# ugadiarov-la-phystech-edu/OCRL

Measured on AMD Instinct MI355X. Metric: images/sec (node) SLATE pretrain 128x128, 6 slots, 3 iters, higher is better.
Workload: dtype f32

## Files before the change

include/ocrl_hip.h:

```cpp
#ifndef OCRL_HIP_H
#define OCRL_HIP_H
#include <stddef.h>

#ifdef __cplusplus
extern "C" {
#endif

#define OCRL_ABI_VERSION 5

const char* ocrl_last_error(void);
int ocrl_abi_version(void);

typedef struct ocrl_slate ocrl_slate;
typedef struct ocrl_slate_config {
    int obs_size, obs_channels;
    int vocab_size, d_model;
    int cnn_hidden;
    int num_slots, num_iterations, slot_size, mlp_hidden;
    int num_dec_blocks, num_dec_heads;
    float dropout;
    int max_batch;
    int use_bcdec;
    int hard;
    int num_slot_heads;
// ... 77 lines not shown
    int accumulate;
} ocrl_conv_wgrad_desc;
size_t ocrl_conv_wgrad_desc_size(void);
int ocrl_conv2d_bwd_weight_ex(const ocrl_conv_wgrad_desc* d, float* ws, size_t ws_floats, void* stream);
int ocrl_layernorm_fwd(const float* x, const float* gamma, const float* beta, float* y, float* mean, float* rstd, long long R, int F, void* stream);
int ocrl_layernorm_bwd(const float* dy, const float* x, const float* mean, const float* rstd, const float* gamma, float* dx, float* dgb,
                       long long R, int F, float* ws, size_t ws_floats, void* stream);

int ocrl_sa_input_plan(long long R, int out[3]);
int ocrl_sa_input_fwd(const float* e4, const float* gamma, const float* beta, const float* W0, const float* b0, const float* W2, const float* b2,
                      float* mean, float* rstd, float* h1, float* x, long long R, int max_wgs, void* stream);
int ocrl_sa_input_bwd(const float* dx, const float* h1, const float* e4, const float* mean, const float* rstd, const float* gamma, const float* beta,
                      const float* W0, const float* W2, float* de4, float* dW0, float* db0, float* dW2, float* db2, float* dgamma, float* dbeta,
                      long long R, int max_wgs, float* ws, size_t ws_floats, void* stream);

int ocrl_attention_fwd(const float* q, const float* k, const float* v, float* o, float* lse, int B, int T, int d, int h, int ld,
                       float p, unsigned long long seed, unsigned site, void* stream);
int ocrl_attention_bwd(const float* q, const float* k, const float* v, const float* o, const float* lse, const float* dO,
                       float* dq, float* dk, float* dv, float* delta, int B, int T, int d, int h, int ld,
                       float p, unsigned long long seed, unsigned site, void* stream);

int ocrl_obs_u8_to_f32(const unsigned char* obs_hwc, float* obs_chw, int B, int H, int W, int C, void* stream);

int ocrl_prof_enable(unsigned tag_mask);
int ocrl_prof_collect(double* ms, long long* count, int ntags);

size_t ocrl_slot_attention_ws_floats(int B, int K, int D, int H, int I);
int ocrl_slot_attention_fwd(const float* x, const float* slots0, const float* const* w, float* slots, float* attn, int B, int N, int K, int D,
                            int H, int I, float* ws, size_t ws_floats, void* stream);
int ocrl_slot_attention_bwd(const float* x, const float* dslots, float* dx, float* dslots0, float* const* dw, int B, int N, int K, int D, int H,
// ... 179 lines not shown
```

ocrl_amd/_lib.py:

```python
import ctypes
import os
from ctypes import POINTER, c_char_p, c_float, c_int, c_longlong, c_size_t, c_uint, c_ulonglong, c_void_p

_HERE = os.path.dirname(os.path.abspath(__file__))
LIB_PATH = os.environ.get("OCRL_HIP_LIB") or os.path.join(_HERE, "libocrl_hip.so")
_lib = None


class SlateConfig(ctypes.Structure):
    _fields_ = [(n, c_int) for n in ("obs_size", "obs_channels", "vocab_size", "d_model", "cnn_hidden", "num_slots",
                                      "num_iterations", "slot_size", "mlp_hidden", "num_dec_blocks", "num_dec_heads")] + \
               [("dropout", c_float), ("max_batch", c_int), ("use_bcdec", c_int), ("hard", c_int), ("num_slot_heads", c_int)]


class IodineConfig(ctypes.Structure):
    _fields_ = [(n, c_int) for n in ("obs_size", "obs_channels", "slot_size", "num_iterations", "num_slots")] + \
               [("sigma", c_float), ("beta", c_float), ("layer_norm", c_int), ("ref_mlp_hidden", c_int), ("max_batch", c_int)]


class GemmDesc(ctypes.Structure):
    _fields_ = [("A", c_void_p), ("B", c_void_p), ("C", c_void_p)] + \
               [(n, c_int) for n in ("M", "N", "K", "lda", "ldb", "ldc", "akc", "bkc", "batch", "batch_inner")] + \
               [(n, c_longlong) for n in ("sA", "sB", "sC", "sAi", "sBi", "sCi")] + \
               [("splitk", c_int), ("alpha", c_float), ("bias", c_void_p), ("relu", c_int),
# ... 122 lines not shown
    L.ocrl_conv2d_wgrad_ws_floats.restype = c_size_t
    L.ocrl_conv2d_bwd_weight.argtypes = [p, p, p, p, c_int, c_int, c_int, c_int, c_int, c_int, p, c_size_t, p]
    L.ocrl_conv_desc_size.restype = c_size_t
    L.ocrl_conv_wgrad_desc_size.restype = c_size_t
    for name, cls in (("ocrl_conv_desc", ConvDesc), ("ocrl_conv_wgrad_desc", ConvWgradDesc)):
        n = getattr(L, name + "_size")()
        if n != ctypes.sizeof(cls):
            raise RuntimeError(f"libocrl_hip.so: {name} is {n} bytes, this binding's {cls.__name__} {ctypes.sizeof(cls)}")
    L.ocrl_conv2d_ex.argtypes = [POINTER(ConvDesc), p, c_size_t, p]
    L.ocrl_conv2d_bwd_weight_ex.argtypes = [POINTER(ConvWgradDesc), p, c_size_t, p]
    L.ocrl_layernorm_fwd.argtypes = [p, p, p, p, p, p, c_longlong, c_int, p]
    L.ocrl_layernorm_bwd.argtypes = [p, p, p, p, p, p, p, c_longlong, c_int, p, c_size_t, p]
    L.ocrl_sa_input_plan.argtypes = [c_longlong, POINTER(c_int * 3)]
    L.ocrl_sa_input_fwd.argtypes = [p] * 11 + [c_longlong, c_int, p]
    L.ocrl_sa_input_bwd.argtypes = [p] * 16 + [c_longlong, c_int, p, c_size_t, p]
    L.ocrl_attention_fwd.argtypes = [p, p, p, p, p, c_int, c_int, c_int, c_int, c_int, c_float, c_ulonglong, c_uint, p]
    L.ocrl_attention_bwd.argtypes = [p, p, p, p, p, p, p, p, p, p, c_int, c_int, c_int, c_int, c_int, c_float, c_ulonglong, c_uint, p]
    L.ocrl_obs_u8_to_f32.argtypes = [p, p, c_int, c_int, c_int, c_int, p]
    L.ocrl_prof_enable.argtypes = [c_uint]
    L.ocrl_prof_collect.argtypes = [POINTER(ctypes.c_double * 8), POINTER(c_longlong * 8), c_int]
    L.ocrl_iodine_create.argtypes = [POINTER(IodineConfig), POINTER(p)]
    L.ocrl_iodine_destroy.argtypes = [p]
    L.ocrl_iodine_destroy.restype = None
    L.ocrl_iodine_param_count.argtypes = [p]
    L.ocrl_iodine_param_info.argtypes = [p, c_int, c_char_p, c_int, POINTER(c_int * 4), POINTER(c_int), POINTER(c_longlong), POINTER(c_longlong)]
    L.ocrl_iodine_flat_size.argtypes = [p]
    L.ocrl_iodine_flat_size.restype = c_longlong
    L.ocrl_iodine_workspace_bytes.argtypes = [p]
    L.ocrl_iodine_workspace_bytes.restype = c_size_t
    L.ocrl_iodine_bind.argtypes = [p, p, p, p, p, p, c_size_t]
# ... 113 lines not shown
```

ocrl_amd/csrc/capi.cpp:

```cpp
#include <stdarg.h>
#include <stdint.h>
#include <string.h>

#include <new>

#include "../../include/ocrl_hip.h"
#include "iodine_model.h"
#include "slate_model.h"

static thread_local char g_err[512] = "";

void ocrl_set_error(const char* fmt, ...) {
    va_list ap;
    va_start(ap, fmt);
    vsnprintf(g_err, sizeof g_err, fmt, ap);
    va_end(ap);
}

template <class M>
struct Handle {
    using Model = M;
    M* m = nullptr;
};
struct ocrl_slate : Handle<SlateModel> {};
// ... 272 lines not shown
    if (!out || R <= 0) { ocrl_set_error("ocrl_sa_input_plan: needs R > 0 and an output array"); return 1; }
    sa_input_plan(R, 0, out);
    return 0;
}
int ocrl_sa_input_fwd(const float* e4, const float* gamma, const float* beta, const float* W0, const float* b0, const float* W2, const float* b2,
                      float* mean, float* rstd, float* h1, float* x, long long R, int max_wgs, void* stream) {
    return sa_input_fwd_launch(e4, gamma, beta, W0, b0, W2, b2, mean, rstd, nullptr, h1, x, R, max_wgs, ST(stream));
}
int ocrl_sa_input_bwd(const float* dx, const float* h1, const float* e4, const float* mean, const float* rstd, const float* gamma, const float* beta,
                      const float* W0, const float* W2, float* de4, float* dW0, float* db0, float* dW2, float* db2, float* dgamma, float* dbeta,
                      long long R, int max_wgs, float* ws, size_t ws_floats, void* stream) {
    return sa_input_bwd_launch(dx, h1, e4, mean, rstd, gamma, beta, W0, W2, de4, dW0, db0, dW2, db2, dgamma, dbeta, R, max_wgs, ws, ws_floats,
                               ST(stream));
}

int ocrl_attention_fwd(const float* q, const float* k, const float* v, float* o, float* lse, int B, int T, int d, int h, int ld, float p,
                       unsigned long long seed, unsigned site, void* stream) {
    AttnArgs a;
    a.q = q; a.k = k; a.v = v; a.o = o; a.lse = lse; a.B = B; a.T = T; a.d = d; a.h = h; a.ld = ld; a.p = p; a.seed = seed; a.site = site;
    return attn_launch(a, 0, ST(stream));
}
int ocrl_attention_bwd(const float* q, const float* k, const float* v, const float* o, const float* lse, const float* dO, float* dq,
                       float* dk, float* dv, float* delta, int B, int T, int d, int h, int ld, float p, unsigned long long seed,
                       unsigned site, void* stream) {
    AttnArgs a;
    a.q = q; a.k = k; a.v = v; a.o = const_cast<float*>(o); a.lse = const_cast<float*>(lse); a.B = B; a.T = T; a.d = d; a.h = h; a.ld = ld;
    a.p = p; a.seed = seed; a.site = site; a.dO = dO; a.dq = dq; a.dk = dk; a.dv = dv; a.delta = delta;
    return attn_launch(a, 1, ST(stream));
}

// ... 37 lines not shown
```

ocrl_amd/csrc/kernels.h:

```cpp
#pragma once
#include "common.h"
#include "../../include/ocrl_hip.h"

enum { PROF_CONV5 = 0, PROF_CONV_OTHER = 1, PROF_WGRAD = 2, PROF_GEMM = 3, PROF_SA_FWD = 4, PROF_SA_BWD = 5, PROF_ATTN_FWD = 6, PROF_ATTN_BWD = 7, PROF_NTAGS = 8 };
int prof_begin(int tag, hipStream_t st);
void prof_end(int idx, hipStream_t st);

struct GemmArgs {
    const float* A = nullptr;
    const float* B = nullptr;
    float* C = nullptr;
    int M = 0, N = 0, K = 0;
    int lda = 0, ldb = 0, ldc = 0;
    int akc = 1, bkc = 1;
    int batch = 1;
    int batch_inner = 1;
    long long sA = 0, sB = 0, sC = 0;
    long long sAi = 0, sBi = 0, sCi = 0;
    int splitk = 1;
    long long sCsplit = 0;
    float alpha = 1.f;
    const float* bias = nullptr;
    int relu = 0;
    float drop_p = 0.f;
// ... 198 lines not shown
int patchify4_launch(const float* in, float* out, int B, int C, int S, hipStream_t st);
int pixel_shuffle_launch(const float* in, float* out, int B, int h, int w, int Cout, int forward, const float* mask, hipStream_t st);
int layernorm_fwd_launch(const float* x, const float* g, const float* b, float* y, float* mean, float* rstd, long long R, int F, hipStream_t st);
int layernorm_bwd_launch(const float* dy, const float* x, const float* mean, const float* rstd, const float* g, float* dx,
                         float* dgb, long long R, int F, int accumulate_dx, int accumulate_dgb, float* ws, size_t ws_floats, hipStream_t st);
int colsum_launch(const float* X, long long ld, float* out, long long R, int F, int accumulate, float scale, float* ws, size_t ws_floats, hipStream_t st);

#define SA_INPUT_SLAB (2 * 4096 + 4 * 64)
void sa_input_plan(long long R, int max_wgs, int out[3]);
int sa_input_fwd_launch(const float* e4, const float* gamma, const float* beta, const float* W0, const float* b0, const float* W2, const float* b2,
                        float* mean, float* rstd, float* ln0, float* h1, float* x, long long R, int max_wgs, hipStream_t st);
int sa_input_bwd_launch(const float* dx, const float* h1, const float* e4, const float* mean, const float* rstd, const float* gamma, const float* beta,
                        const float* W0, const float* W2, float* de4, float* dW0, float* db0, float* dW2, float* db2, float* dgamma, float* dbeta,
                        long long R, int max_wgs, float* ws, size_t ws_floats, hipStream_t st);
int reduce_partials_launch(const float* part, int n, float* out, float scale, int accumulate, hipStream_t st);
int mse_launch(const float* obs, const float* recon, float* drecon, float* out, int B, int C, int H, int W, float* ws, size_t ws_floats, hipStream_t st);
int gumbel_softmax_launch(const float* raw, const float* e1, const float* e2, float* z, int* tokens, long long R, int V, float tau,
                          unsigned long long seed, hipStream_t st, float* zst = nullptr);
int softmax_bwd_rows_launch(const float* z, float* d, long long R, int V, float scale, hipStream_t st);
int softmax_stat_combine_launch(const float* stat, int nseg, long long R, float* lse, const float* hstat, const int* hidx, int* tokens,
                                const float* pred, int ldp, const int* tok, float* out, float scale, float* ws, size_t ws_floats, hipStream_t st,
                                const float* cdf_scores = nullptr, int cdf_V = 0, float cdf_tau = 1.f, unsigned long long cdf_seed = 0);
int exp_rows_launch(const float* y, const float* lse, float* z, long long R, int V, hipStream_t st);
int rowdot_bias64_launch(const float* g, const float* act, const float* bias, long long R, float* out, hipStream_t st);
int embed_fwd_launch(const int* tokens, const float* dict, const float* bos, const float* pe, float* out, int B, int T, int d, float p,
                     unsigned long long seed, hipStream_t st);
size_t embed_bwd_ws_floats(long long BT, int V, int d);
int embed_bwd_launch(float* g, const int* tokens, float* ddict, int B, int T, int V, int d, float p, unsigned long long seed, float* ws,
                     size_t ws_floats, hipStream_t st);
int dropout_apply_launch(const float* x, float* y, long long n, float p, unsigned long long seed, unsigned site, hipStream_t st);
// ... 177 lines not shown
```

ocrl_amd/csrc/slate_model.cpp:

```cpp
#include "slate_model.h"

#include <stdlib.h>
#include <functional>
#include <utility>

#include <math.h>
#include <stdarg.h>
#include <string.h>

static std::string fmt(const char* f, ...) {
    char buf[256];
    va_list ap;
    va_start(ap, f);
    vsnprintf(buf, sizeof buf, f, ap);
    va_end(ap);
    return buf;
}

SlateModel::SlateModel(const SlateConfig& c) : cfg(c) {
    S = c.obs_size; E = S / 4; T = E * E; N = S * S; V = c.vocab; d = c.d_model; C = c.cnn_hidden;
    K = c.num_slots; I = c.num_iters; D = c.slot_size; H = c.mlp_hidden; NB = c.num_blocks; NH = c.num_heads;
    DH = d / NH; Bmax = c.max_batch; SH = c.slot_heads > 0 ? c.slot_heads : 1;
    const int ch = c.obs_channels;
    add_param("_dvae._encoder.0.m.weight", {64, ch, 4, 4}, 0); add_param("_dvae._encoder.0.m.bias", {64}, 0);
// ... 229 lines not shown
            OCRL_HIP(hipEventCreateWithFlags(&ev_fork_, hipEventDisableTiming));
            OCRL_HIP(hipEventCreateWithFlags(&ev_join_, hipEventDisableTiming));
            OCRL_HIP(hipEventCreateWithFlags(&ev_tokens_, hipEventDisableTiming));
            const char* w = getenv("OCRL_DW_SIDE");
            dw_mode_ = (overlap_mode_ >= 3 && !cfg.use_bcdec) ? (w ? atoi(w) : 2) : 0;
            if (dw_mode_) {
                for (hipEvent_t& ev : ev_dw_) OCRL_HIP(hipEventCreateWithFlags(&ev, hipEventDisableTiming));
                OCRL_HIP(hipEventCreateWithFlags(&ev_join2_, hipEventDisableTiming));
                if (dw_mode_ == 2) OCRL_HIP(hipStreamCreateWithFlags(&side2_, hipStreamNonBlocking));
            }
        }
    }
    {
        const char* e = getenv("OCRL_SA_INPUT");
        sa_input_ = e ? atoi(e) : 1;
    }
    {
        const char* e = getenv("OCRL_XATTN");
        xattn_ = !cfg.use_bcdec && xattn_supported(K, d, NH) && (e ? atoi(e) != 0 : true);
        if (!cfg.use_bcdec && xa_zero_floats_) OCRL_HIP(hipMemset(xa_zero_base_, 0, xa_zero_floats_ * sizeof(float)));
    }
    RC(posgrid_launch(gridT_, S, 0));
    RC(fill_launch(recon_, (long long)Bmax * N * 4, 0.f, 0));
    const SaWts wo = sa_wts_layout(C, D, H);
    const std::string sa = "_slotattn.slot_attention.";
    std::vector<PackEntry> ent;
    auto e = [&](const std::string& name, int rows, int cols, int off, int tr) {
        PackEntry x; x.src = P(name); x.rows = rows; x.cols = cols; x.dst_off = off; x.transpose = tr;
        ent.push_back(x);
    };
// ... 151 lines not shown
        a.A = zraw_; a.B = P("_dvae._decoder.0.m.weight"); a.C = dd0_; a.M = (int)BT; a.N = 64; a.K = V; a.lda = V; a.ldb = V; a.ldc = 64;
        a.bias = P("_dvae._decoder.0.m.bias"); a.relu = 1; a.a_mode = 2; a.x_lse = zlse_;
        RC(gemm_launch(a, st));
    } else {
    if (!zin) zin = zdec_;
    RC(lin_fwd(zin, V, P("_dvae._decoder.0.m.weight"), P("_dvae._decoder.0.m.bias"), dd0_, 64, BT, 64, V, 1, nullptr, 0, 0.f, 0, st));
    }
    RC(conv_layer_fwd(dd0_, dw_fwd_[0], P("_dvae._decoder.1.m.bias"), dd1_, B, E, E, 3, 64, 1, nullptr, nullptr, st));
    RC(lin_fwd(dd1_, 64, P("_dvae._decoder.2.m.weight"), P("_dvae._decoder.2.m.bias"), dd2_, 64, BT, 64, 64, 1, nullptr, 0, 0.f, 0, st));
    RC(lin_fwd(dd2_, 64, P("_dvae._decoder.3.m.weight"), P("_dvae._decoder.3.m.bias"), dd3_, 64, BT, 64, 64, 1, nullptr, 0, 0.f, 0, st));
    RC(lin_fwd(dd3_, 64, P("_dvae._decoder.4.m.weight"), P("_dvae._decoder.4.m.bias"), dd4_, 256, BT, 256, 64, 1, nullptr, 0, 0.f, 0, st));
    RC(pixel_shuffle_launch(dd4_, ps1_, B, E, E, 64, 1, nullptr, st));
    RC(conv_layer_fwd(ps1_, dw_fwd_[1], P("_dvae._decoder.6.m.bias"), dd6_, B, 2 * E, 2 * E, 3, 64, 1, nullptr, nullptr, st));
    RC(lin_fwd(dd6_, 64, P("_dvae._decoder.7.m.weight"), P("_dvae._decoder.7.m.bias"), dd7_, 64, 4 * BT, 64, 64, 1, nullptr, 0, 0.f, 0, st));
    RC(lin_fwd(dd7_, 64, P("_dvae._decoder.8.m.weight"), P("_dvae._decoder.8.m.bias"), dd8_, 64, 4 * BT, 64, 64, 1, nullptr, 0, 0.f, 0, st));
    RC(lin_fwd(dd8_, 64, P("_dvae._decoder.9.m.weight"), P("_dvae._decoder.9.m.bias"), dd9_, 256, 4 * BT, 256, 64, 1, nullptr, 0, 0.f, 0, st));
    RC(pixel_shuffle_launch(dd9_, ps2_, B, 2 * E, 2 * E, 64, 1, nullptr, st));
    RC(lin_fwd(ps2_, 64, P("_dvae._decoder.11.weight"), P("_dvae._decoder.11.bias"), recon_, 4, BN, ch, 64, 0, nullptr, 0, 0.f, 0, st));
    RC(mse_launch(last_.obs, recon_, drecon, metrics_ + (drecon ? 0 : 4), B, ch, S, S, scratch_, scratch_floats_, st));
    return 0;
}

int SlateModel::fwd_decoder(hipStream_t st, bool with_ce) {
    const int B = last_.B;
    const long long BT = (long long)B * T;
    const float p = pdrop_;
    const float scale = 1.0f / sqrtf((float)DH);
    RC(lin_fwd(slots_, D, P("_slotproj.weight"), nullptr, mem_, d, (long long)B * K, d, D, 0, nullptr, 0, 0.f, 0, st));
    RC(embed_fwd_launch(tokens_, P("_dict.dictionary.weight"), P("_bos_token._bos_token"), P("_z_pos.pe"), emb_, B, T, d, p, last_.seed, st));
    bool fold_pending = false;
    if (xattn_) {
        XaFoldHost f;
        f.mem = mem_; f.B = B; f.K = K; f.d = d; f.h = NH; f.nblk = NB;
// ... 452 lines not shown
    RC(conv_layer_wgrad(e1_, gB_, G("_enc._encoder.1.m.weight"), G("_enc._encoder.1.m.bias"), B, S, S, 5, 64, 64, st));
    RC(conv_layer_fwd(gB_, cw_bwd_[1], nullptr, gA_, B, S, S, 5, 64, 0, nullptr, e1_, st));
    {
        const int ch = cfg.obs_channels, ldc0 = (25 * ch + 3) & ~3;
        if (!side_w) RC(im2col5_launch(obs8_, col0_, BN, S, S, ch, ldc0, st));
        RC(lin_bwd_w(gA_, 64, col0_, ldc0, dw0p_, G("_enc._encoder.0.m.bias"), BN, 64, ldc0, 1.f, st));
        RC(unpack5_launch(dw0p_, G("_enc._encoder.0.m.weight"), ch, ldc0, st));
    }
    return 0;
}

int SlateModel::bwd_dvae(hipStream_t st) {
    const int B = last_.B;
    const long long BT = (long long)B * T, BN = (long long)B * N;
    const int ch = cfg.obs_channels;
    float* w4 = scratch_ + scratch_floats_ - 1024;
    {
        GemmArgs a;
        a.A = drecon_; a.B = ps2_; a.C = w4; a.M = 4; a.N = 64; a.K = (int)BN; a.lda = 4; a.ldb = 64; a.ldc = 64; a.akc = 0; a.bkc = 0;
        long long splits = BN / 512; if (splits > 512) splits = 512; if (splits < 1) splits = 1;
        if (splits > 1) {
            a.splitk = (int)splits; a.C = scratch_; a.sCsplit = 256;
            RC(gemm_launch(a, st));
            RC(splitk_reduce_launch(scratch_, w4, 256, (int)splits, 256, 0, st));
        } else RC(gemm_launch(a, st));
        RC(copy_launch(w4, G("_dvae._decoder.11.weight"), ch * 64, st));
        RC(colsum_launch(drecon_, 4, w4 + 256, BN, 4, 0, 1.f, scratch_, scratch_floats_ - 1024, st));
        RC(copy_launch(w4 + 256, G("_dvae._decoder.11.bias"), ch, st));
    }
    RC(lin_bwd_x(drecon_, 4, w11p_, gdA_, 64, BN, 4, 64, nullptr, 0, nullptr, 0, st));
    RC(pixel_shuffle_launch(gdA_, gdB_, B, 2 * E, 2 * E, 64, 0, dd9_, st));
    RC(lin_bwd_w(gdB_, 256, dd8_, 64, G("_dvae._decoder.9.m.weight"), G("_dvae._decoder.9.m.bias"), 4 * BT, 256, 64, 1.f, st));
    RC(lin_bwd_x(gdB_, 256, P("_dvae._decoder.9.m.weight"), gdA_, 64, 4 * BT, 256, 64, dd8_, 64, nullptr, 0, st));
    RC(lin_bwd_w(gdA_, 64, dd7_, 64, G("_dvae._decoder.8.m.weight"), G("_dvae._decoder.8.m.bias"), 4 * BT, 64, 64, 1.f, st));
    RC(lin_bwd_x(gdA_, 64, P("_dvae._decoder.8.m.weight"), gdB_, 64, 4 * BT, 64, 64, dd7_, 64, nullptr, 0, st));
    RC(lin_bwd_w(gdB_, 64, dd6_, 64, G("_dvae._decoder.7.m.weight"), G("_dvae._decoder.7.m.bias"), 4 * BT, 64, 64, 1.f, st));
    RC(lin_bwd_x(gdB_, 64, P("_dvae._decoder.7.m.weight"), gdA_, 64, 4 * BT, 64, 64, dd6_, 64, nullptr, 0, st));
    RC(conv_layer_wgrad(ps1_, gdA_, G("_dvae._decoder.6.m.weight"), G("_dvae._decoder.6.m.bias"), B, 2 * E, 2 * E, 3, 64, 64, st));
    RC(conv_layer_fwd(gdA_, dw_bwd_[1], nullptr, gdB_, B, 2 * E, 2 * E, 3, 64, 0, nullptr, ps1_, st));
    RC(pixel_shuffle_launch(gdB_, gdA_, B, E, E, 64, 0, nullptr, st));
    RC(lin_bwd_w(gdA_, 256, dd3_, 64, G("_dvae._decoder.4.m.weight"), G("_dvae._decoder.4.m.bias"), BT, 256, 64, 1.f, st));
    RC(lin_bwd_x(gdA_, 256, P("_dvae._decoder.4.m.weight"), gdB_, 64, BT, 256, 64, dd3_, 64, nullptr, 0, st));
    RC(lin_bwd_w(gdB_, 64, dd2_, 64, G("_dvae._decoder.3.m.weight"), G("_dvae._decoder.3.m.bias"), BT, 64, 64, 1.f, st));
    RC(lin_bwd_x(gdB_, 64, P("_dvae._decoder.3.m.weight"), gdA_, 64, BT, 64, 64, dd2_, 64, nullptr, 0, st));
    RC(lin_bwd_w(gdA_, 64, dd1_, 64, G("_dvae._decoder.2.m.weight"), G("_dvae._decoder.2.m.bias"), BT, 64, 64, 1.f, st));
    RC(lin_bwd_x(gdA_, 64, P("_dvae._decoder.2.m.weight"), gdB_, 64, BT, 64, 64, dd1_, 64, nullptr, 0, st));
    RC(conv_layer_wgrad(dd0_, gdB_, G("_dvae._decoder.1.m.weight"), G("_dvae._decoder.1.m.bias"), B, E, E, 3, 64, 64, st));
    RC(conv_layer_fwd(gdB_, dw_bwd_[0], nullptr, gdA_, B, E, E, 3, 64, 0, nullptr, dd0_, st));
// ... 156 lines not shown
```

ocrl_amd/csrc/slate_model.h:

```cpp
#pragma once
#include <map>
#include <string>
#include <vector>

#include "kernels.h"
#include "model_base.h"

struct SlateConfig {
    int obs_size = 64, obs_channels = 3, vocab = 4096, d_model = 192, cnn_hidden = 64;
    int num_slots = 5, num_iters = 3, slot_size = 192, mlp_hidden = 192;
    int num_blocks = 4, num_heads = 4;
    float dropout = 0.1f;
    int max_batch = 1;
    int use_bcdec = 0;
    int hard = 0;
    int slot_heads = 1;
};

struct StepInputs {
    const float* obs = nullptr;
    int B = 0;
    float tau = 1.f;
    int train = 1;
    unsigned long long seed = 0;
// ... 82 lines not shown
    PackEntry* sa_pack_dev_ = nullptr;
    int sa_pack_n_ = 0, sa_pack_max_ = 0;
    float *cw_fwd_[4], *cw_bwd_[4];
    int conv_x3_ = -1;
    std::map<const float*, const float*> x3_of_;
    float *dw_fwd_[2], *dw_bwd_[2];
    float *w11p_;
    float *mem_, *emb_;
    struct Blk {
        float *ln1, *ln1_mean, *ln1_rstd, *q, *k, *v, *lse, *ao, *x1;
        float *ln2, *ln2_mean, *ln2_rstd, *cq, *ck, *cv, *cP, *cao, *x2;
        float *ln3, *ln3_mean, *ln3_rstd, *f1, *x3;
        float *xaAb, *xaAbT, *xaVo, *xaVoT;
    };
    int sa_input_ = 1;
    bool xattn_ = false;
    float *xa_dAb_ = nullptr, *xa_dVo_ = nullptr, *xa_pq_ = nullptr, *xa_po_ = nullptr;
    size_t xa_zero_floats_ = 0;
    float* xa_zero_base_ = nullptr;
    std::vector<Blk> blk_;
    struct BlkG { float *gbr[3], *gf1, *gt2, *gqkv, *xaPd, *xaDs; };
    std::vector<BlkG> bg_;
    struct EncGraph { hipGraphExec_t exec = nullptr; int warm = 0; };
    std::map<int, EncGraph> enc_graphs_;
    int enc_graph_mode_ = -1;
    hipStream_t cap_ = nullptr;
    float* obs_stage_ = nullptr;
    unsigned long long* seed_dev_ = nullptr;
    int dw_mode_ = 0;
    hipStream_t side2_ = nullptr;
// ... 16 lines not shown
```

Before: 1728.

## Fuse dVAE decoder tail (1x1 conv, pixel shuffle, output conv) fwd and bwd

Adds fused MFMA kernels for the final dVAE decoder stages. The forward pass computes the 64→256 linear with ReLU, the pixel shuffle and the 64→3 output projection in one persistent kernel, writing dd9 and recon directly. The backward pass fuses the output-conv gradient, the pixel-unshuffle, the ReLU mask, dW9/db9/dW11/db11 partials and the dx gradient, then reduces per-workgroup slabs in a second kernel. This removes separate GEMM launches and the ps2/gdB intermediate round-trips through global memory, at the cost of complex hand-written tiling and extra scratch space for the slabs.

```diff
diff --git a/include/ocrl_hip.h b/include/ocrl_hip.h
--- a/include/ocrl_hip.h
+++ b/include/ocrl_hip.h
@@ -115,6 +115,13 @@
                       const float* W0, const float* W2, float* de4, float* dW0, float* db0, float* dW2, float* db2, float* dgamma, float* dbeta,
                       long long R, int max_wgs, float* ws, size_t ws_floats, void* stream);
 
+int ocrl_dvae_tail_plan(long long R, int out[3]);
+int ocrl_dvae_tail_fwd(const float* dd8, const float* W9, const float* b9, const float* W11, const float* b11, float* dd9, float* recon,
+                       int B, int h, int w, int max_wgs, void* stream);
+int ocrl_dvae_tail_bwd(const float* drecon, const float* dd9, const float* dd8, const float* W11p, const float* W9, float* ddd8, float* dW9,
+                       float* db9, float* dW11, float* db11, int B, int h, int w, int max_wgs, float* ws, size_t ws_floats, void* stream);
+int ocrl_pixel_shuffle(const float* in, float* out, int B, int h, int w, int Cout, int forward, const float* mask, void* stream);
+
 int ocrl_attention_fwd(const float* q, const float* k, const float* v, float* o, float* lse, int B, int T, int d, int h, int ld,
                        float p, unsigned long long seed, unsigned site, void* stream);
 int ocrl_attention_bwd(const float* q, const float* k, const float* v, const float* o, const float* lse, const float* dO,
diff --git a/ocrl_amd/_lib.py b/ocrl_amd/_lib.py
--- a/ocrl_amd/_lib.py
+++ b/ocrl_amd/_lib.py
@@ -160,6 +160,10 @@
     L.ocrl_sa_input_plan.argtypes = [c_longlong, POINTER(c_int * 3)]
     L.ocrl_sa_input_fwd.argtypes = [p] * 11 + [c_longlong, c_int, p]
     L.ocrl_sa_input_bwd.argtypes = [p] * 16 + [c_longlong, c_int, p, c_size_t, p]
+    L.ocrl_dvae_tail_plan.argtypes = [c_longlong, POINTER(c_int * 3)]
+    L.ocrl_dvae_tail_fwd.argtypes = [p] * 7 + [c_int] * 4 + [p]
+    L.ocrl_dvae_tail_bwd.argtypes = [p] * 10 + [c_int] * 4 + [p, c_size_t, p]
+    L.ocrl_pixel_shuffle.argtypes = [p, p, c_int, c_int, c_int, c_int, c_int, p, p]
     L.ocrl_attention_fwd.argtypes = [p, p, p, p, p, c_int, c_int, c_int, c_int, c_int, c_float, c_ulonglong, c_uint, p]
     L.ocrl_attention_bwd.argtypes = [p, p, p, p, p, p, p, p, p, p, c_int, c_int, c_int, c_int, c_int, c_float, c_ulonglong, c_uint, p]
     L.ocrl_obs_u8_to_f32.argtypes = [p, p, c_int, c_int, c_int, c_int, p]
diff --git a/ocrl_amd/csrc/capi.cpp b/ocrl_amd/csrc/capi.cpp
--- a/ocrl_amd/csrc/capi.cpp
+++ b/ocrl_amd/csrc/capi.cpp
@@ -310,6 +310,24 @@
                                ST(stream));
 }
 
+int ocrl_dvae_tail_plan(long long R, int out[3]) {
+    if (!out || R <= 0) { ocrl_set_error("ocrl_dvae_tail_plan: needs R > 0 and an output array"); return 1; }
+    dvae_tail_plan(R, 0, out);
+    return 0;
+}
+int ocrl_dvae_tail_fwd(const float* dd8, const float* W9, const float* b9, const float* W11, const float* b11, float* dd9, float* recon,
+                       int B, int h, int w, int max_wgs, void* stream) {
+    return dvae_tail_fwd_launch(dd8, W9, b9, W11, b11, dd9, recon, B, h, w, max_wgs, ST(stream));
+}
+int ocrl_dvae_tail_bwd(const float* drecon, const float* dd9, const float* dd8, const float* W11p, const float* W9, float* ddd8, float* dW9,
+                       float* db9, float* dW11, float* db11, int B, int h, int w, int max_wgs, float* ws, size_t ws_floats, void* stream) {
+    return dvae_tail_bwd_launch(drecon, dd9, dd8, W11p, W9, ddd8, dW9, db9, dW11, db11, B, h, w, max_wgs, ws, ws_floats, ST(stream));
+}
+int ocrl_pixel_shuffle(const float* in, float* out, int B, int h, int w, int Cout, int forward, const float* mask, void* stream) {
+    if (!in || !out || B <= 0 || h <= 0 || w <= 0 || Cout <= 0) { ocrl_set_error("ocrl_pixel_shuffle: needs in, out and positive B, h, w, Cout"); return 1; }
+    return pixel_shuffle_launch(in, out, B, h, w, Cout, forward, mask, ST(stream));
+}
+
 int ocrl_attention_fwd(const float* q, const float* k, const float* v, float* o, float* lse, int B, int T, int d, int h, int ld, float p,
                        unsigned long long seed, unsigned site, void* stream) {
     AttnArgs a;
diff --git a/ocrl_amd/csrc/dvae_tail.hip b/ocrl_amd/csrc/dvae_tail.hip
--- /dev/null
+++ b/ocrl_amd/csrc/dvae_tail.hip
@@ -0,0 +1,374 @@
+#include "common.h"
+#include "kernels.h"
+
+#define DVT_TR 64
+#define DVT_XLD 68
+#define DVT_FLD 36
+#define DVT_FPL (64 * DVT_FLD + 8)
+#define DVT_BLD 65
+#define DVT_BPL (64 * DVT_BLD + 8)
+#define DVT_FWD_MAX_WGS 512
+#define DVT_BWD_MAX_WGS 256
+
+__device__ __forceinline__ float4 dvt_ld4(const float* __restrict__ p, long long row, long long R, int ld, int c4) {
+    const float4 v = *reinterpret_cast<const float4*>(p + (row < R ? row : R - 1) * ld + c4 * 4);
+    return row < R ? v : make_float4(0.f, 0.f, 0.f, 0.f);
+}
+__device__ __forceinline__ long long dvt_pixel(long long row, int w, int i, int j) {
+    const long long yy = row / w;
+    return (2 * yy + i) * (2LL * w) + 2 * (row - yy * w) + j;
+}
+__device__ __forceinline__ float4 dvt_ld_pix(const float* __restrict__ p, long long row, long long R, int w, int i, int j) {
+    const float4 v = *reinterpret_cast<const float4*>(p + dvt_pixel(row < R ? row : R - 1, w, i, j) * 4);
+    return row < R ? v : make_float4(0.f, 0.f, 0.f, 0.f);
+}
+#define DVT_ROW(r, lh) (((r) & 3) + 8 * ((r) >> 2) + 4 * (lh))
+
+__global__ __launch_bounds__(256, 2) void dvae_tail_fwd_kernel(const float* __restrict__ dd8, const float* __restrict__ W9, const float* __restrict__ b9,
+                                                               const float* __restrict__ W11, const float* __restrict__ b11,
+                                                               float* __restrict__ dd9, float* __restrict__ recon, long long R, int w) {
+    __shared__ __attribute__((aligned(16))) float At[DVT_TR * DVT_XLD], Ht[4 * DVT_FPL], W11s[4 * 64];
+    const int t = threadIdx.x, lane = t & 63, wv = t >> 6, c4 = lane & 15, rsub = lane >> 4;
+    const int li = lane & 31, lh = lane >> 5;
+    float w9f[2][8][4], b9v[2];
+#pragma unroll
+    for (int p = 0; p < 2; ++p) {
+#pragma unroll
+        for (int c = 0; c < 8; ++c) {
+            const float4 a = *reinterpret_cast<const float4*>(W9 + (p * 128 + wv * 32 + li) * 64 + c * 8 + 4 * lh);
+            w9f[p][c][0] = a.x; w9f[p][c][1] = a.y; w9f[p][c][2] = a.z; w9f[p][c][3] = a.w;
+        }
+        b9v[p] = b9[p * 128 + wv * 32 + li];
+    }
+    W11s[t] = t < 192 ? W11[t] : 0.f;
+    const float b11v = li < 3 ? b11[li] : 0.f;
+    const long long ntiles = (R + DVT_TR - 1) / DVT_TR;
+    const int lr0 = wv * 16 + rsub;
+    float4 v[4];
+#pragma unroll
+    for (int i = 0; i < 4; ++i) v[i] = dvt_ld4(dd8, (long long)blockIdx.x * DVT_TR + lr0 + 4 * i, R, 64, c4);
+    for (long long tile = blockIdx.x; tile < ntiles; tile += gridDim.x) {
+        const long long r0 = tile * DVT_TR;
+#pragma unroll
+        for (int i = 0; i < 4; ++i) *reinterpret_cast<float4*>(At + (lr0 + 4 * i) * DVT_XLD + c4 * 4) = v[i];
+#pragma unroll
+        for (int i = 0; i < 4; ++i) v[i] = dvt_ld4(dd8, (tile + gridDim.x) * DVT_TR + lr0 + 4 * i, R, 64, c4);
+        __syncthreads();
+        f32x16 r11[2];
+#pragma unroll
+        for (int r = 0; r < 16; ++r) { r11[0][r] = 0.f; r11[1][r] = 0.f; }
+#pragma unroll
+        for (int p = 0; p < 2; ++p) {
+            f32x16 a0, a1;
+#pragma unroll
+            for (int r = 0; r < 16; ++r) { a0[r] = 0.f; a1[r] = 0.f; }
+#pragma unroll
+            for (int c = 0; c < 8; ++c) {
+                const float4 x0 = *reinterpret_cast<const float4*>(At + li * DVT_XLD + c * 8 + 4 * lh);
+                const float4 x1 = *reinterpret_cast<const float4*>(At + (32 + li) * DVT_XLD + c * 8 + 4 * lh);
+                a0 = __builtin_amdgcn_mfma_f32_32x32x2f32(x0.x, w9f[p][c][0], a0, 0, 0, 0);
+                a1 = __builtin_amdgcn_mfma_f32_32x32x2f32(x1.x, w9f[p][c][0], a1, 0, 0, 0);
+                a0 = __builtin_amdgcn_mfma_f32_32x32x2f32(x0.y, w9f[p][c][1], a0, 0, 0, 0);
+                a1 = __builtin_amdgcn_mfma_f32_32x32x2f32(x1.y, w9f[p][c][1], a1, 0, 0, 0);
+                a0 = __builtin_amdgcn_mfma_f32_32x32x2f32(x0.z, w9f[p][c][2], a0, 0, 0, 0);
+                a1 = __builtin_amdgcn_mfma_f32_32x32x2f32(x1.z, w9f[p][c][2], a1, 0, 0, 0);
+                a0 = __builtin_amdgcn_mfma_f32_32x32x2f32(x0.w, w9f[p][c][3], a0, 0, 0, 0);
+                a1 = __builtin_amdgcn_mfma_f32_32x32x2f32(x1.w, w9f[p][c][3], a1, 0, 0, 0);
+            }
+            {
+                float* const hp = Ht + (li & 3) * DVT_FPL + wv * 8 + (li >> 2);
+#pragma unroll
+                for (int r = 0; r < 16; ++r) {
+                    const int row = DVT_ROW(r, lh);
+                    hp[row * DVT_FLD] = fmaxf(a0[r] + b9v[p], 0.f);
+                    hp[(32 + row) * DVT_FLD] = fmaxf(a1[r] + b9v[p], 0.f);
+                }
+            }
+            __syncthreads();
+            {
+                const int cl = t & 31;
+#pragma unroll
+                for (int i = 0; i < 8; ++i) {
+                    const int row = (t >> 5) + 8 * i;
+                    const float* const hp = Ht + row * DVT_FLD + cl;
+                    const float4 o = make_float4(hp[0], hp[DVT_FPL], hp[2 * DVT_FPL], hp[3 * DVT_FPL]);
+                    if (r0 + row < R) *reinterpret_cast<float4*>(dd9 + (r0 + row) * 256 + p * 128 + cl * 4) = o;
+                }
+            }
+#pragma unroll
+            for (int cl = 0; cl < 4; ++cl) {
+                float4 bw = make_float4(0.f, 0.f, 0.f, 0.f);
+                if (li < 4) bw = *reinterpret_cast<const float4*>(W11s + li * 64 + (4 * p + cl) * 8 + 4 * lh);
+                const float4 x0 = *reinterpret_cast<const float4*>(Ht + wv * DVT_FPL + li * DVT_FLD + cl * 8 + 4 * lh);
+                const float4 x1 = *reinterpret_cast<const float4*>(Ht + wv * DVT_FPL + (32 + li) * DVT_FLD + cl * 8 + 4 * lh);
+                r11[0] = __builtin_amdgcn_mfma_f32_32x32x2f32(x0.x, bw.x, r11[0], 0, 0, 0);
+                r11[1] = __builtin_amdgcn_mfma_f32_32x32x2f32(x1.x, bw.x, r11[1], 0, 0, 0);
+                r11[0] = __builtin_amdgcn_mfma_f32_32x32x2f32(x0.y, bw.y, r11[0], 0, 0, 0);
+                r11[1] = __builtin_amdgcn_mfma_f32_32x32x2f32(x1.y, bw.y, r11[1], 0, 0, 0);
+                r11[0] = __builtin_amdgcn_mfma_f32_32x32x2f32(x0.z, bw.z, r11[0], 0, 0, 0);
+                r11[1] = __builtin_amdgcn_mfma_f32_32x32x2f32(x1.z, bw.z, r11[1], 0, 0, 0);
+                r11[0] = __builtin_amdgcn_mfma_f32_32x32x2f32(x0.w, bw.w, r11[0], 0, 0, 0);
+                r11[1] = __builtin_amdgcn_mfma_f32_32x32x2f32(x1.w, bw.w, r11[1], 0, 0, 0);
+            }
+            __syncthreads();
+        }
+        if (li < 4) {
+#pragma unroll
+            for (int r = 0; r < 16; ++r) {
+                const int row = DVT_ROW(r, lh);
+                At[(wv * 64 + row) * 4 + li] = li < 3 ? r11[0][r] + b11v : 0.f;
+                At[(wv * 64 + 32 + row) * 4 + li] = li < 3 ? r11[1][r] + b11v : 0.f;
+            }
+        }
+        __syncthreads();
+        {
+            const int i = t >> 7, rl = (t & 127) >> 1, j = t & 1;
+            if (r0 + rl < R)
+                *reinterpret_cast<float4*>(recon + dvt_pixel(r0 + rl, w, i, j) * 4) = *reinterpret_cast<const float4*>(At + ((2 * i + j) * 64 + rl) * 4);
+        }
+        __syncthreads();
+    }
+}
+
+template <bool DX>
+__device__ __forceinline__ void dvt_bwd_tiles(const float* __restrict__ drecon, const float* __restrict__ dd9, const float* __restrict__ dd8,
+                                              const float* __restrict__ W11p, float* __restrict__ ddd8, float* __restrict__ sl, long long R, int w,
+                                              float* __restrict__ G, float* __restrict__ X, float* __restrict__ DR, const float* __restrict__ W9s,
+                                              f32x16& dW11a, float& db9a, float4& db11a) {
+    const int t = threadIdx.x, lane = t & 63, wv = t >> 6, li = lane & 31, lh = lane >> 5;
+    const int sp = wv >> 1, cb = wv & 1;
+    float wb[4];
+#pragma unroll
+    for (int j = 0; j < 4; ++j) wb[j] = lh == 0 ? W11p[j * 64 + cb * 32 + li] : 0.f;
+    f32x16 dW9a[DX ? 1 : 4];
+    if (!DX) {
+#pragma unroll
+        for (int q = 0; q < (DX ? 1 : 4); ++q)
+#pragma unroll
+            for (int r = 0; r < 16; ++r) dW9a[q][r] = 0.f;
+    }
+    const long long ntiles = (R + DVT_TR - 1) / DVT_TR;
+    const int gc = t & 63, gr = t >> 6, xc = t & 15, xr = t >> 4;
+    const int pi = (t >> 7) & 1, prl = (t & 127) >> 1, pj = t & 1;
+    float4 n9[8], n8[2], ndr;
+#pragma unroll
+    for (int i = 0; i < 8; ++i) n9[i] = dvt_ld4(dd9, (long long)blockIdx.x * DVT_TR + gr + 8 * i, R, 256, gc);
+#pragma unroll
+    for (int i = 0; i < 2; ++i) n8[i] = dvt_ld4(dd8, (long long)blockIdx.x * DVT_TR + xr + 32 * i, R, 64, xc);
+    ndr = dvt_ld_pix(drecon, (long long)blockIdx.x * DVT_TR + prl, R, w, pi, pj);
+    for (long long tile = blockIdx.x; tile < ntiles; tile += gridDim.x) {
+        const long long r0 = tile * DVT_TR;
+        __syncthreads();
+#pragma unroll
+        for (int i = 0; i < 8; ++i) {
+            float* const gp = G + (gr + 8 * i) * DVT_BLD + gc;
+            gp[0] = n9[i].x; gp[DVT_BPL] = n9[i].y; gp[2 * DVT_BPL] = n9[i].z; gp[3 * DVT_BPL] = n9[i].w;
+        }
+#pragma unroll
+        for (int i = 0; i < 2; ++i) *reinterpret_cast<float4*>(X + (xr + 32 * i) * DVT_XLD + xc * 4) = n8[i];
+        if (DX) {
+            *reinterpret_cast<float4*>(DR + ((2 * pi + pj) * 64 + prl) * 4) = ndr;
+            db11a.x += ndr.x; db11a.y += ndr.y; db11a.z += ndr.z; db11a.w += ndr.w;
+        }
+        {
+            const long long rn = (tile + gridDim.x) * DVT_TR;
+#pragma unroll
+            for (int i = 0; i < 8; ++i) n9[i] = dvt_ld4(dd9, rn + gr + 8 * i, R, 256, gc);
+#pragma unroll
+            for (int i = 0; i < 2; ++i) n8[i] = dvt_ld4(dd8, rn + xr + 32 * i, R, 64, xc);
+            if (DX) ndr = dvt_ld_pix(drecon, rn + prl, R, w, pi, pj);
+        }
+        __syncthreads();
+        {
+            float* const gp = G + sp * DVT_BPL + cb * 32 + li;
+            const float* const dp = DR + sp * 256;
+#pragma unroll 2
+            for (int c = 0; c < 8; ++c) {
+                float fa[4], fb[4];
+#pragma unroll
+                for (int j = 0; j < 4; ++j) {
+                    const int row = c * 8 + 4 * lh + j;
+                    fa[j] = li < 4 ? dp[row * 4 + li] : 0.f;
+                    fb[j] = gp[row * DVT_BLD];
+                }
+#pragma unroll
+                for (int j = 0; j < 4; ++j) dW11a = __builtin_amdgcn_mfma_f32_32x32x2f32(fa[j], fb[j], dW11a, 0, 0, 0);
+            }
+#pragma unroll
+            for (int rb = 0; rb < 2; ++rb) {
+                float4 a = make_float4(0.f, 0.f, 0.f, 0.f);
+                if (lh == 0) a = *reinterpret_cast<const float4*>(dp + (rb * 32 + li) * 4);
+                f32x16 acc;
+#pragma unroll
+                for (int r = 0; r < 16; ++r) acc[r] = 0.f;
+                acc = __builtin_amdgcn_mfma_f32_32x32x2f32(a.x, wb[0], acc, 0, 0, 0);
+                acc = __builtin_amdgcn_mfma_f32_32x32x2f32(a.y, wb[1], acc, 0, 0, 0);
+                acc = __builtin_amdgcn_mfma_f32_32x32x2f32(a.z, wb[2], acc, 0, 0, 0);
+                acc = __builtin_amdgcn_mfma_f32_32x32x2f32(a.w, wb[3], acc, 0, 0, 0);
+#pragma unroll
+                for (int r = 0; r < 16; ++r) {
+                    float* const q = gp + (rb * 32 + DVT_ROW(r, lh)) * DVT_BLD;
+                    const float g = *q > 0.f ? acc[r] : 0.f;
+                    *q = g;
+                    db9a += g;
+                }
+            }
+        }
+        __syncthreads();
+        if (DX) {
+            const int rb = wv >> 1, cb2 = wv & 1;
+            const float* const ga = G + (rb * 32 + li) * DVT_BLD + lh;
+            const float* const wk = W9s + (4 * lh) * 64 + cb2 * 32 + li;
+            f32x16 acc;
+#pragma unroll
+            for (int r = 0; r < 16; ++r) acc[r] = 0.f;
+#pragma unroll 4
+            for (int cc = 0; cc < 32; ++cc) {
+                const float a0 = ga[2 * cc], a1 = ga[DVT_BPL + 2 * cc], a2 = ga[2 * DVT_BPL + 2 * cc], a3 = ga[3 * DVT_BPL + 2 * cc];
+                acc = __builtin_amdgcn_mfma_f32_32x32x2f32(a0, wk[(8 * cc) * 64], acc, 0, 0, 0);
+                acc = __builtin_amdgcn_mfma_f32_32x32x2f32(a1, wk[(8 * cc + 1) * 64], acc, 0, 0, 0);
+                acc = __builtin_amdgcn_mfma_f32_32x32x2f32(a2, wk[(8 * cc + 2) * 64], acc, 0, 0, 0);
+                acc = __builtin_amdgcn_mfma_f32_32x32x2f32(a3, wk[(8 * cc + 3) * 64], acc, 0, 0, 0);
+            }
+#pragma unroll
+            for (int r = 0; r < 16; ++r) {
+                const int row = rb * 32 + DVT_ROW(r, lh);
+                const float mk = X[row * DVT_XLD + cb2 * 32 + li];
+                float v = acc[r];
+                v = mk > 0.f ? v : 0.f * v * (mk + 1.f);
+                if (r0 + row < R) ddd8[(r0 + row) * 64 + cb2 * 32 + li] = v;
+            }
+        } else {
+            const float* const g0 = G + (li & 3) * DVT_BPL + (2 * (wv - 4)) * 8 + (li >> 2);
+#pragma unroll 2
+            for (int c = 0; c < 8; ++c) {
+                float fa[4], fc[4], fb[4], fd[4];
+#pragma unroll
+                for (int j = 0; j < 4; ++j) {
+                    const int row = c * 8 + 4 * lh + j;
+                    fa[j] = g0[row * DVT_BLD];
+                    fc[j] = g0[row * DVT_BLD + 8];
+                    fb[j] = X[row * DVT_XLD + li];
+                    fd[j] = X[row * DVT_XLD + 32 + li];
+                }
+#pragma unroll
+                for (int j = 0; j < 4; ++j) {
+                    dW9a[0] = __builtin_amdgcn_mfma_f32_32x32x2f32(fa[j], fb[j], dW9a[0], 0, 0, 0);
+                    dW9a[DX ? 0 : 1] = __builtin_amdgcn_mfma_f32_32x32x2f32(fa[j], fd[j], dW9a[DX ? 0 : 1], 0, 0, 0);
+                    dW9a[DX ? 0 : 2] = __builtin_amdgcn_mfma_f32_32x32x2f32(fc[j], fb[j], dW9a[DX ? 0 : 2], 0, 0, 0);
+                    dW9a[DX ? 0 : 3] = __builtin_amdgcn_mfma_f32_32x32x2f32(fc[j], fd[j], dW9a[DX ? 0 : 3], 0, 0, 0);
+                }
+            }
+        }
+    }
+    if (!DX) {
+        const int u = wv - 4;
+#pragma unroll
+        for (int q = 0; q < (DX ? 1 : 4); ++q)
+#pragma unroll
+            for (int r = 0; r < 16; ++r) sl[((2 * u + (q >> 1)) * 32 + DVT_ROW(r, lh)) * 64 + (q & 1) * 32 + li] = dW9a[q][r];
+    }
+}
+
+__global__ __launch_bounds__(512, 1) void dvae_tail_bwd_kernel(const float* __restrict__ drecon, const float* __restrict__ dd9, const float* __restrict__ dd8,
+                                                               const float* __restrict__ W11p, const float* __restrict__ W9,
+                                                               float* __restrict__ ddd8, float* __restrict__ slab, long long R, int w) {
+    __shared__ __attribute__((aligned(16))) float G[4 * DVT_BPL], X[DVT_TR * DVT_XLD], DR[4 * 64 * 4], W9s[256 * 64];
+    const int t = threadIdx.x, lane = t & 63, wv = t >> 6, li = lane & 31, lh = lane >> 5;
+    const int sp = wv >> 1, cb = wv & 1;
+#pragma unroll
+    for (int i = 0; i < 8; ++i)
+        *reinterpret_cast<float4*>(W9s + (t + 512 * i) * 4) = *reinterpret_cast<const float4*>(W9 + (t + 512 * i) * 4);
+    f32x16 dW11a;
+#pragma unroll
+    for (int r = 0; r < 16; ++r) dW11a[r] = 0.f;
+    float db9a = 0.f;
+    float4 db11a = make_float4(0.f, 0.f, 0.f, 0.f);
+    float* const sl = slab + (size_t)blockIdx.x * DVAE_TAIL_SLAB;
+    if (__builtin_amdgcn_readfirstlane(wv) < 4) dvt_bwd_tiles<true>(drecon, dd9, dd8, W11p, ddd8, sl, R, w, G, X, DR, W9s, dW11a, db9a, db11a);
+    else dvt_bwd_tiles<false>(drecon, dd9, dd8, W11p, ddd8, sl, R, w, G, X, DR, W9s, dW11a, db9a, db11a);
+    __syncthreads();
+    float* const rb9 = G;
+    float* const rw11 = G + 512;
+    float* const rb11 = G + 512 + 1024;
+    rb9[(wv * 2 + lh) * 32 + li] = db9a;
+    if (lh == 0) {
+#pragma unroll
+        for (int o = 0; o < 4; ++o) rw11[(sp * 4 + o) * 64 + cb * 32 + li] = dW11a[o];
+    }
+    if (t < 256) *reinterpret_cast<float4*>(rb11 + t * 4) = db11a;
+    __syncthreads();
+    if (t < 256) {
+        const int c = t >> 2, s = t & 3, wq = 2 * s + (c >> 5);
+        sl[16384 + t] = rb9[(wq * 2) * 32 + (c & 31)] + rb9[(wq * 2 + 1) * 32 + (c & 31)];
+    } else {
+        const int idx = t - 256;
+        sl[16640 + idx] = (rw11[idx] + rw11[256 + idx]) + (rw11[512 + idx] + rw11[768 + idx]);
+    }
+    for (int half = 128; half >= 1; half >>= 1) {
+        if (t < half) {
+            float4 a = *reinterpret_cast<const float4*>(rb11 + t * 4);
+            const float4 b = *reinterpret_cast<const float4*>(rb11 + (t + half) * 4);
+            a.x += b.x; a.y += b.y; a.z += b.z; a.w += b.w;
+            *reinterpret_cast<float4*>(rb11 + t * 4) = a;
+        }
+        __syncthreads();
+    }
+    if (t < 32) sl[16896 + t] = t < 4 ? rb11[t] : 0.f;
+}
+
+__global__ __launch_bounds__(256) void dvae_tail_reduce_kernel(const float* __restrict__ slab, int nslab, float* __restrict__ dW9, float* __restrict__ db9,
+                                                               float* __restrict__ dW11, float* __restrict__ db11) {
+    __shared__ float red[8][32];
+    const int ci = threadIdx.x & 31, grp = threadIdx.x >> 5, col = blockIdx.x * 32 + ci;
+    const int per = (nslab + 7) / 8, s0 = grp * per, s1 = min(nslab, s0 + per);
+    float a = 0.f;
+    for (int s = s0; s < s1; ++s) a += slab[(size_t)s * DVAE_TAIL_SLAB + col];
+    red[grp][ci] = a;
+    __syncthreads();
+    if (threadIdx.x < 32) {
+        float v = red[0][ci];
+#pragma unroll
+        for (int k = 1; k < 8; ++k) v += red[k][ci];
+        if (col < 16384) dW9[col] = v;
+        else if (col < 16640) db9[col - 16384] = v;
+        else if (col < 16640 + 192) dW11[col - 16640] = v;
+        else if (col >= 16896 && col < 16899) db11[col - 16896] = v;
+    }
+}
+
+void dvae_tail_plan(long long R, int max_wgs, int out[3]) {
+    const long long ntiles = (R + DVT_TR - 1) / DVT_TR;
+    long long wgs = max_wgs > 0 && max_wgs < DVT_BWD_MAX_WGS ? max_wgs : DVT_BWD_MAX_WGS;
+    if (wgs > ntiles) wgs = ntiles;
+    out[0] = DVT_TR; out[1] = (int)wgs; out[2] = DVAE_TAIL_SLAB;
+}
+
+int dvae_tail_fwd_launch(const float* dd8, const float* W9, const float* b9, const float* W11, const float* b11, float* dd9, float* recon,
+                         int B, int h, int w, int max_wgs, hipStream_t st) {
+    OCRL_REQUIRE(B > 0 && h > 0 && w > 0, "dvae_tail_fwd: no rows");
+    OCRL_REQUIRE(dd8 && W9 && b9 && W11 && b11 && dd9 && recon, "dvae_tail_fwd: null argument");
+    OCRL_REQUIRE(aligned16(dd8, W9, dd9, recon), "dvae_tail_fwd: tensors must be 16-byte aligned");
+    const long long R = (long long)B * h * w, ntiles = (R + DVT_TR - 1) / DVT_TR;
+    long long wgs = max_wgs > 0 && max_wgs < DVT_FWD_MAX_WGS ? max_wgs : DVT_FWD_MAX_WGS;
+    if (wgs > ntiles) wgs = ntiles;
+    hipLaunchKernelGGL(dvae_tail_fwd_kernel, dim3((unsigned)wgs), dim3(256), 0, st, dd8, W9, b9, W11, b11, dd9, recon, R, w);
+    OCRL_CHECK_LAUNCH("dvae_tail_fwd");
+    return 0;
+}
+
+int dvae_tail_bwd_launch(const float* drecon, const float* dd9, const float* dd8, const float* W11p, const float* W9, float* ddd8, float* dW9,
+                         float* db9, float* dW11, float* db11, int B, int h, int w, int max_wgs, float* ws, size_t ws_floats, hipStream_t st) {
+    OCRL_REQUIRE(B > 0 && h > 0 && w > 0, "dvae_tail_bwd: no rows");
+    OCRL_REQUIRE(drecon && dd9 && dd8 && W11p && W9 && ddd8 && dW9 && db9 && dW11 && db11 && ws, "dvae_tail_bwd: null argument");
+    OCRL_REQUIRE(aligned16(drecon, dd9, dd8, W9, ws), "dvae_tail_bwd: tensors must be 16-byte aligned");
+    const long long R = (long long)B * h * w;
+    int plan[3];
+    dvae_tail_plan(R, max_wgs, plan);
+    OCRL_REQUIRE((size_t)plan[1] * DVAE_TAIL_SLAB <= ws_floats, "dvae_tail_bwd: workspace too small (%d slabs of %d floats)", plan[1], DVAE_TAIL_SLAB);
+    hipLaunchKernelGGL(dvae_tail_bwd_kernel, dim3(plan[1]), dim3(512), 0, st, drecon, dd9, dd8, W11p, W9, ddd8, ws, R, w);
+    OCRL_CHECK_LAUNCH("dvae_tail_bwd");
+    hipLaunchKernelGGL(dvae_tail_reduce_kernel, dim3(DVAE_TAIL_SLAB / 32), dim3(256), 0, st, ws, plan[1], dW9, db9, dW11, db11);
+    OCRL_CHECK_LAUNCH("dvae_tail_reduce");
+    return 0;
+}
diff --git a/ocrl_amd/csrc/kernels.h b/ocrl_amd/csrc/kernels.h
--- a/ocrl_amd/csrc/kernels.h
+++ b/ocrl_amd/csrc/kernels.h
@@ -236,6 +236,13 @@
                         const float* W0, const float* W2, float* de4, float* dW0, float* db0, float* dW2, float* db2, float* dgamma, float* dbeta,
                         long long R, int max_wgs, float* ws, size_t ws_floats, hipStream_t st);
 int reduce_partials_launch(const float* part, int n, float* out, float scale, int accumulate, hipStream_t st);
+
+#define DVAE_TAIL_SLAB (256 * 64 + 256 + 4 * 64 + 32)
+void dvae_tail_plan(long long R, int max_wgs, int out[3]);
+int dvae_tail_fwd_launch(const float* dd8, const float* W9, const float* b9, const float* W11, const float* b11, float* dd9, float* recon,
+                         int B, int h, int w, int max_wgs, hipStream_t st);
+int dvae_tail_bwd_launch(const float* drecon, const float* dd9, const float* dd8, const float* W11p, const float* W9, float* ddd8, float* dW9,
+                         float* db9, float* dW11, float* db11, int B, int h, int w, int max_wgs, float* ws, size_t ws_floats, hipStream_t st);
 int mse_launch(const float* obs, const float* recon, float* drecon, float* out, int B, int C, int H, int W, float* ws, size_t ws_floats, hipStream_t st);
 int gumbel_softmax_launch(const float* raw, const float* e1, const float* e2, float* z, int* tokens, long long R, int V, float tau,
                           unsigned long long seed, hipStream_t st, float* zst = nullptr);
diff --git a/ocrl_amd/csrc/slate_model.cpp b/ocrl_amd/csrc/slate_model.cpp
--- a/ocrl_amd/csrc/slate_model.cpp
+++ b/ocrl_amd/csrc/slate_model.cpp
@@ -267,6 +267,10 @@
     {
         const char* e = getenv("OCRL_SA_INPUT");
         sa_input_ = e ? atoi(e) : 1;
+    }
+    {
+        const char* e = getenv("OCRL_DVAE_TAIL");
+        dvae_tail_ = e ? atoi(e) : 1;
     }
     {
         const char* e = getenv("OCRL_XATTN");
@@ -448,9 +452,14 @@
     RC(conv_layer_fwd(ps1_, dw_fwd_[1], P("_dvae._decoder.6.m.bias"), dd6_, B, 2 * E, 2 * E, 3, 64, 1, nullptr, nullptr, st));
     RC(lin_fwd(dd6_, 64, P("_dvae._decoder.7.m.weight"), P("_dvae._decoder.7.m.bias"), dd7_, 64, 4 * BT, 64, 64, 1, nullptr, 0, 0.f, 0, st));
     RC(lin_fwd(dd7_, 64, P("_dvae._decoder.8.m.weight"), P("_dvae._decoder.8.m.bias"), dd8_, 64, 4 * BT, 64, 64, 1, nullptr, 0, 0.f, 0, st));
+    if (dvae_tail_) {
+        RC(dvae_tail_fwd_launch(dd8_, P("_dvae._decoder.9.m.weight"), P("_dvae._decoder.9.m.bias"), P("_dvae._decoder.11.weight"),
+                                P("_dvae._decoder.11.bias"), dd9_, recon_, B, 2 * E, 2 * E, 0, st));
+    } else {
     RC(lin_fwd(dd8_, 64, P("_dvae._decoder.9.m.weight"), P("_dvae._decoder.9.m.bias"), dd9_, 256, 4 * BT, 256, 64, 1, nullptr, 0, 0.f, 0, st));
     RC(pixel_shuffle_launch(dd9_, ps2_, B, 2 * E, 2 * E, 64, 1, nullptr, st));
     RC(lin_fwd(ps2_, 64, P("_dvae._decoder.11.weight"), P("_dvae._decoder.11.bias"), recon_, 4, BN, ch, 64, 0, nullptr, 0, 0.f, 0, st));
+    }
     RC(mse_launch(last_.obs, recon_, drecon, metrics_ + (drecon ? 0 : 4), B, ch, S, S, scratch_, scratch_floats_, st));
     return 0;
 }
@@ -933,6 +942,15 @@
     const int B = last_.B;
     const long long BT = (long long)B * T, BN = (long long)B * N;
     const int ch = cfg.obs_channels;
+    if (dvae_tail_) {
+        int plan[3];
+        dvae_tail_plan(4 * BT, 0, plan);
+        const size_t slabs = (scratch_floats_ - 1024) / DVAE_TAIL_SLAB;
+        OCRL_REQUIRE(scratch_floats_ > 1024 && slabs >= 1, "bwd_dvae: scratch too small for the decoder-tail slabs");
+        RC(dvae_tail_bwd_launch(drecon_, dd9_, dd8_, w11p_, P("_dvae._decoder.9.m.weight"), gdA_, G("_dvae._decoder.9.m.weight"),
+                                G("_dvae._decoder.9.m.bias"), G("_dvae._decoder.11.weight"), G("_dvae._decoder.11.bias"), B, 2 * E, 2 * E,
+                                slabs < (size_t)plan[1] ? (int)slabs : 0, scratch_, scratch_floats_ - 1024, st));
+    } else {
     float* w4 = scratch_ + scratch_floats_ - 1024;
     {
         GemmArgs a;
@@ -951,6 +969,7 @@
     RC(pixel_shuffle_launch(gdA_, gdB_, B, 2 * E, 2 * E, 64, 0, dd9_, st));
     RC(lin_bwd_w(gdB_, 256, dd8_, 64, G("_dvae._decoder.9.m.weight"), G("_dvae._decoder.9.m.bias"), 4 * BT, 256, 64, 1.f, st));
     RC(lin_bwd_x(gdB_, 256, P("_dvae._decoder.9.m.weight"), gdA_, 64, 4 * BT, 256, 64, dd8_, 64, nullptr, 0, st));
+    }
     RC(lin_bwd_w(gdA_, 64, dd7_, 64, G("_dvae._decoder.8.m.weight"), G("_dvae._decoder.8.m.bias"), 4 * BT, 64, 64, 1.f, st));
     RC(lin_bwd_x(gdA_, 64, P("_dvae._decoder.8.m.weight"), gdB_, 64, 4 * BT, 64, 64, dd7_, 64, nullptr, 0, st));
     RC(lin_bwd_w(gdB_, 64, dd6_, 64, G("_dvae._decoder.7.m.weight"), G("_dvae._decoder.7.m.bias"), 4 * BT, 64, 64, 1.f, st));
diff --git a/ocrl_amd/csrc/slate_model.h b/ocrl_amd/csrc/slate_model.h
--- a/ocrl_amd/csrc/slate_model.h
+++ b/ocrl_amd/csrc/slate_model.h
@@ -120,6 +120,7 @@
         float *xaAb, *xaAbT, *xaVo, *xaVoT;
     };
     int sa_input_ = 1;
+    int dvae_tail_ = 1;
     bool xattn_ = false;
     float *xa_dAb_ = nullptr, *xa_dVo_ = nullptr, *xa_pq_ = nullptr, *xa_po_ = nullptr;
     size_t xa_zero_floats_ = 0;
```

Result: no change. 1744, median of 6 (+0.9%).
